# victorca25/traiNNer

Measured on AMD Instinct MI355X. Metric: HR images/sec (G+D step), ESRGAN x4 128->512, higher is better.
Workload: dtype f32 (bf16x3)

## Files before the change

### trainner_amd/csrc/wgrad_tile.hip

```cpp
#include <type_traits>
#include <utility>
#include "common.h"

namespace {

struct WgJob {
    const float *x; const float *g; float *ws; float *dbp;
    int x_ct, x_co, Cin, g_ct, g_co, Cout;
    int KoutP, KinVP;
    int cinp32;
    int ncib, job_begin;
};
struct WgK {
    int N, H, W, Ho, Wo;
    int tiles_x, tiles_y, tiles_total, tiles_per_split, nsplits, njobs;
    int bf;
    int reflect;
    WgJob job[TNR_WGRAD_GROUP_MAX];
};

template <int A_T, int B_T, int NTAPS_>
struct WgCfg {
    static constexpr int AB = A_T * B_T;
    static constexpr int KS = (NTAPS_ == 9 && (AB == 1 || AB == 2)) ? 4 / AB : 1;
// ... 102 lines not shown
        t_boff[j] = (ty * WT + tx) * CIB + bb * 32;
    }

    f32x16 acc[J];
#pragma unroll
    for (int j = 0; j < J; ++j)
#pragma unroll
        for (int r = 0; r < 16; ++r) acc[j][r] = 0.f;
    float bsum = 0.f;
    const bool want_bias = (a.dbp != nullptr) && (cib == 0);

    const int t_begin = split * a.tiles_per_split;
    int t_end = t_begin + a.tiles_per_split;
    if (t_end > a.tiles_total) t_end = a.tiles_total;

    constexpr int G_ITEMS = PX * (COB / 4), G_IT = (G_ITEMS + 255) / 256;
    constexpr int X_ITEMS = HT * WT * (CIB / 4), X_IT = (X_ITEMS + 255) / 256;
    constexpr int N_IT = G_IT + X_IT;
    constexpr int BATCH = (PIPE || N_IT <= 12) ? N_IT : 8;
    constexpr int NBATCH = (N_IT + BATCH - 1) / BATCH;
    f32x4 rr[BATCH];
    struct TileAt { int n, ty0, tx0; };
    auto tile_at = [&](int tile) __attribute__((always_inline)) {
        int q = tile;
        const int tx = q % a.tiles_x;
        q /= a.tiles_x;
        const int ty = q % a.tiles_y;
        return TileAt{q / a.tiles_y, ty * THG, tx * TWG};
    };
    auto load_item = [&](const TileAt &ta, int batch, auto kc) __attribute__((always_inline)) {
        constexpr int k = decltype(kc)::value;
        const int n = ta.n, ty0 = ta.ty0, tx0 = ta.tx0;
        {
            const int it = batch * BATCH + k;
            f32x4 v = {0.f, 0.f, 0.f, 0.f};
            if (it < G_IT) {
                const int i = tid + it * 256;
                const int p = i / (COB / 4), c4 = i - p * (COB / 4);
                const int r = p / TWG, c = p - r * TWG;
                const int oy = ty0 + r, ox = tx0 + c;
                const int co = cob * COB + c4 * 4;
                if (i < G_ITEMS && oy < a.Ho && ox < a.Wo && co < a.Cout) {
                    const int off = ((n * a.Ho + oy) * a.Wo + ox) * a.g_ct + a.g_co + co;
                    v = *reinterpret_cast<const f32x4 *>(a.g + off);
                }
            } else if (it < N_IT) {
                const int i = tid + (it - G_IT) * 256;
                const int pix = i / (CIB / 4), c4 = i - pix * (CIB / 4);
                const int hr = pix / WT, hc = pix - hr * WT;
                const int vb = cib * B_T + (c4 >> 3);
                int Y, X, c;
                bool ok;
                if (S2D) {
                    const int nb32 = a.cinp32 >> 5;
                    const int pp = vb / nb32;
                    c = (vb - pp * nb32) * 32 + (c4 & 7) * 4;
                    Y = 2 * (ty0 + hr) - 1 + (pp >> 1);
                    X = 2 * (tx0 + hc) - 1 + (pp & 1);
                    ok = (pp < 4) & (Y >= 0) & (Y < a.H) & (X >= 0) & (X < a.W);
                } else if (UP) {
                    c = vb * 32 + (c4 & 7) * 4;
                    Y = ty0 + hr - 1;
                    X = tx0 + hc - 1;
                    ok = (Y >= 0) & (Y < 2 * a.H) & (X >= 0) & (X < 2 * a.W);
                    Y >>= 1;
                    X >>= 1;
                } else {
                    c = vb * 32 + (c4 & 7) * 4;
                    Y = ty0 + hr - 1;
                    X = tx0 + hc - 1;
                    if (a.reflect) {
                        Y = Y < 0 ? -Y : (Y >= a.H ? 2 * a.H - 2 - Y : Y);
                        X = X < 0 ? -X : (X >= a.W ? 2 * a.W - 2 - X : X);
                    }
                    ok = (Y >= 0) & (Y < a.H) & (X >= 0) & (X < a.W);
                }
                if (i < X_ITEMS && ok && c < a.Cin) {
                    const int off = ((n * a.H + Y) * a.W + X) * a.x_ct + a.x_co + c;
                    v = *reinterpret_cast<const f32x4 *>(a.x + off);
                }
            }
            rr[k] = v;
        }
    };
    auto load_batch = [&](int tile, int batch) __attribute__((always_inline)) {
        const TileAt ta = tile_at(tile);
        wg_static_for<0, BATCH>([&](auto kc) __attribute__((always_inline)) { load_item(ta, batch, kc); });
    };
#if defined(TNR_WG_SPREAD_ALL) && !defined(TNR_NO_LOAD_SPREAD)
    constexpr bool SPREAD = PIPE;
#else
    constexpr bool SPREAD = false;
#endif
    constexpr int SPREAD_N = 3, IPG = (BATCH + SPREAD_N - 1) / SPREAD_N;
    auto load_group = [&](int tile, auto gc) __attribute__((always_inline)) {
        constexpr int g = decltype(gc)::value;
        constexpr int k0 = g * IPG < BATCH ? g * IPG : BATCH, k1 = (g + 1) * IPG < BATCH ? (g + 1) * IPG : BATCH;
        const TileAt ta = tile_at(tile);
        wg_static_for<k0, k1>([&](auto kc) __attribute__((always_inline)) { load_item(ta, 0, kc); });
    };
    auto split4 = [&](const f32x4 v, wg_f32x2 (&out)[3]) {
        wg_bf16x4 h, m, l;
#pragma unroll
        for (int i = 0; i < 4; ++i) {
            const __bf16 hh = (__bf16)v[i];
            const float r1 = v[i] - (float)hh;
            const __bf16 mm = (__bf16)r1;
            h[i] = hh;
            m[i] = mm;
            l[i] = (__bf16)(r1 - (float)mm);
        }
        out[0] = __builtin_bit_cast(wg_f32x2, h);
        out[1] = __builtin_bit_cast(wg_f32x2, m);
        out[2] = __builtin_bit_cast(wg_f32x2, l);
    };
    char *const s_gb = reinterpret_cast<char *>(smem);
    char *const s_xb = s_gb + (size_t)PX * COB * 6;
    auto store_batch = [&](int batch) {
#pragma unroll
        for (int k = 0; k < BATCH; ++k) {
            const int it = batch * BATCH + k;
            if constexpr (BF == 2) {
                wg_f32x2 pc[3];
                if (it < G_IT) {
                    const int i = tid + it * 256;
                    if (i < G_ITEMS) {
                        split4(rr[k], pc);
                        char *d = s_gb + wg_x3_off(i / (COB / 4), (i % (COB / 4)) * 4, COB);
#pragma unroll
                        for (int sp = 0; sp < 3; ++sp) *reinterpret_cast<wg_f32x2 *>(d + 256 * sp) = pc[sp];
                    }
                } else if (it < N_IT) {
                    const int i = tid + (it - G_IT) * 256;
                    if (i < X_ITEMS) {
                        split4(rr[k], pc);
                        char *d = s_xb + wg_x3_off(i / (CIB / 4), (i % (CIB / 4)) * 4, CIB);
#pragma unroll
                        for (int sp = 0; sp < 3; ++sp) *reinterpret_cast<wg_f32x2 *>(d + 256 * sp) = pc[sp];
                    }
                }
                continue;
            }
            if (it < G_IT) {
                const int i = tid + it * 256;
                if (i < G_ITEMS) *reinterpret_cast<f32x4 *>(s_g + i * 4) = rr[k];
            } else if (it < N_IT) {
                const int i = tid + (it - G_IT) * 256;
                if (i < X_ITEMS) *reinterpret_cast<f32x4 *>(s_x + i * 4) = rr[k];
            }
        }
    };

    if constexpr (DB) {
        static_assert(BF == 2 && MODE == TNR_CONV_3x3 && WPS == 1, "pipelined form: bf16x3, plain 3x3, one workgroup per CU");
        constexpr int WTP = 20;
        constexpr int G_BYTES = PX * COB * 6, X_BYTES = HT * WTP * CIB * 6, TILES_BYTES = G_BYTES + X_BYTES;
        constexpr int SET_BYTES = TILES_BYTES + 3072;
        constexpr int XBLK = (CIB / 32) * 768, GBLK = (COB / 32) * 768;
        constexpr int NP = (J + 1) / 2, MPR = 6 * J, NM = ROWS * MPR;
        constexpr int G0 = NM - 5 * N_IT - 6;
        static_assert(G0 >= 2 * N_IT, "the phase is too short for the staging plan");
        char *const lds = reinterpret_cast<char *>(smem);
        const __amdgpu_buffer_rsrc_t g_rs = __builtin_amdgcn_make_buffer_rsrc(const_cast<float *>(a.g), 0,
                                                                              (int)((unsigned)a.N * a.Ho * a.Wo * a.g_ct * 4u), 0x00020000);
        const __amdgpu_buffer_rsrc_t x_rs = __builtin_amdgcn_make_buffer_rsrc(const_cast<float *>(a.x), 0,
                                                                              (int)((unsigned)a.N * a.H * a.W * a.x_ct * 4u), 0x00020000);
        int it_src[N_IT], it_yx[N_IT], it_dst[N_IT];
#pragma unroll
        for (int k = 0; k < N_IT; ++k) {
            if (k < G_IT) {
                const int i = tid + k * 256;
                const int pp = i / (COB / 4), c4 = i - pp * (COB / 4);
                const int r = pp / TWG, cc = pp - r * TWG;
                const int co = cob * COB + c4 * 4;
                const bool v = i < G_ITEMS && co < a.Cout;
                it_src[k] = v ? (r * a.Wo + cc) * a.g_ct + a.g_co + co : -1;
                it_yx[k] = r | (cc << 8);
                it_dst[k] = i < G_ITEMS ? wg_x3_off(pp, c4 * 4, COB) : TILES_BYTES + tid * 8;
            } else {
                const int i = tid + (k - G_IT) * 256;
                const int pix = i / (CIB / 4), c4 = i - pix * (CIB / 4);
                const int hr = pix / WT, hc = pix - hr * WT;
                const int ch = (cib * B_T + (c4 >> 3)) * 32 + (c4 & 7) * 4;
                const bool v = i < X_ITEMS && ch < a.Cin;
                it_src[k] = v ? ((hr - 1) * a.W + (hc - 1)) * a.x_ct + a.x_co + ch : (1 << 30);
                it_yx[k] = hr | (hc << 8);
                it_dst[k] = i < X_ITEMS ? G_BYTES + wg_x3_off(hr * WTP + hc, c4 * 4, CIB) : TILES_BYTES + tid * 8;
            }
        }
        int ld_ty0 = 0, ld_tx0 = 0, ld_gbase = 0, ld_xbase = 0;
        bool ld_valid = true;
        int l_n = 0, l_ty = 0, l_tx = 0;
        auto load_setup_first = [&](int tile) __attribute__((always_inline)) {
            const TileAt ta = tile_at(tile);
            l_n = ta.n; l_ty = ta.ty0 / THG; l_tx = ta.tx0 / TWG;
        };
        auto load_setup_next = [&]() __attribute__((always_inline)) {
            if (++l_tx == a.tiles_x) {
                l_tx = 0;
                if (++l_ty == a.tiles_y) {
                    l_ty = 0;
                    ++l_n;
                }
            }
        };
        auto load_setup = [&]() __attribute__((always_inline)) {
            ld_ty0 = l_ty * THG; ld_tx0 = l_tx * TWG;
            ld_gbase = ((l_n * a.Ho + ld_ty0) * a.Wo + ld_tx0) * a.g_ct;
            ld_xbase = ((l_n * a.H + ld_ty0) * a.W + ld_tx0) * a.x_ct;
        };
        auto item_load = [&](auto kc) __attribute__((always_inline)) {
            constexpr int k = decltype(kc)::value;
            const int y = it_yx[k] & 255, xx = it_yx[k] >> 8;
            if constexpr (k < G_IT) {
                const bool ok = ld_valid & (it_src[k] >= 0) & (ld_ty0 + y < a.Ho) & (ld_tx0 + xx < a.Wo);
                const unsigned bo = ok ? (unsigned)(ld_gbase + it_src[k]) * 4u : 0xfffffff0u;
                rr[k] = __builtin_bit_cast(f32x4, __builtin_amdgcn_raw_buffer_load_b128(g_rs, (int)bo, 0, 0));
            } else {
                const int Y = ld_ty0 + y - 1, X = ld_tx0 + xx - 1;
                const bool ok = ld_valid & (it_src[k] != (1 << 30)) & ((unsigned)Y < (unsigned)a.H) & ((unsigned)X < (unsigned)a.W);
                const unsigned bo = ok ? (unsigned)(ld_xbase + it_src[k]) * 4u : 0xfffffff0u;
                rr[k] = __builtin_bit_cast(f32x4, __builtin_amdgcn_raw_buffer_load_b128(x_rs, (int)bo, 0, 0));
            }
        };
        wg_bf16x4 ih, im, il;
        f32x4 ir;
        auto item_step = [&](auto kc, auto sc, char *set) __attribute__((always_inline)) {
            constexpr int k = decltype(kc)::value, st = decltype(sc)::value;
            if constexpr (st == 0) {
#if WG_PK_SPLIT
                wg_pk_level(rr[k], ih, ir);
#else
                ih = __builtin_convertvector(rr[k], wg_bf16x4);
                ir = rr[k] - __builtin_convertvector(ih, f32x4);
#endif
            } else if constexpr (st == 1) {
#if WG_PK_SPLIT
                const f32x4 r1 = ir;
                wg_pk_level(r1, im, ir);
#else
                im = __builtin_convertvector(ir, wg_bf16x4);
                ir = ir - __builtin_convertvector(im, f32x4);
#endif
            } else {
#if WG_PK_SPLIT
                if constexpr (st == 2) {
                    const wg_f32x2 a = {ir[0], ir[1]}, b = {ir[2], ir[3]};
                    il = __builtin_bit_cast(wg_bf16x4, wg_f32x2{__builtin_bit_cast(float, __builtin_convertvector(a, wg_bf16x2)),
                                                                __builtin_bit_cast(float, __builtin_convertvector(b, wg_bf16x2))});
                }
#else
                if constexpr (st == 2) il = __builtin_convertvector(ir, wg_bf16x4);
#endif
                *reinterpret_cast<wg_f32x2 *>(set + it_dst[k] + 256 * (st - 2)) = __builtin_bit_cast(wg_f32x2, st == 2 ? ih : (st == 3 ? im : il));
            }
        };
        const int cg = (lane >> 4) & 1, m4 = (lane >> 2) & 3, q4 = lane & 3;
        const int lch = 16 * cg + 4 * q4;
        const int ga_off = ((pg * ROWS * 4 + 2 * half) * (COB / 32) + aa_w) * 768 + m4 * 64 + lch * 2;
        int xb_off[J];
#pragma unroll
        for (int j = 0; j < J; ++j) {
            const int tap = t_tap[j] >> 10, bb = t_tap[j] & 31;
            const int ty = tap / KH, tx = tap - ty * KH;
            const int q0 = tx + 8 * half + m4;
            xb_off[j] = G_BYTES + ((pg * ROWS + ty) * (WTP / 4) + (q0 >> 2)) * XBLK + (q0 & 3) * 64 + bb * 768 + lch * 2;
        }
        constexpr int TA[6] = {0, 2, 1, 0, 1, 0}, TB[6] = {2, 0, 1, 1, 0, 0};
        auto rd = [&](const char *base, int imm) __attribute__((always_inline)) {
            return __builtin_amdgcn_ds_read_tr16_b64_v4i16((wg_lds_s16x4 *)(base + imm));
        };
        typedef short s16x8 __attribute__((ext_vector_type(8)));
        static_assert(J == 9 && WPG == AB, "every wave owns the 9 taps of one (cout half, cin block) pair: tile j = tap j");
        wg_s16x4 ra[2][3][2], rbx[3][3][3][2];
        auto pack = [&](const wg_s16x4 lo4, const wg_s16x4 hi4) __attribute__((always_inline)) {
            const s16x8 v = {lo4[0], lo4[1], lo4[2], lo4[3], hi4[0], hi4[1], hi4[2], hi4[3]};
            return __builtin_bit_cast(wg_bf16x8, v);
        };

        if (t_begin < t_end) {
            load_setup_first(t_begin);
            load_setup();
            wg_static_for<0, N_IT>([&](auto kc) __attribute__((always_inline)) { item_load(kc); });
            wg_static_for<0, N_IT>([&](auto kc) __attribute__((always_inline)) {
                wg_static_for<0, 5>([&](auto sc) __attribute__((always_inline)) { item_step(kc, sc, lds); });
            });
            __syncthreads();
        }
        for (int tile = t_begin; tile < t_end; ++tile) {
            const int cur = (tile - t_begin) & 1;
            const char *set = lds + cur * SET_BYTES;
            char *oset = lds + (cur ^ 1) * SET_BYTES;
            ld_valid = tile + 1 < t_end;
            if (ld_valid) load_setup_next();
            load_setup();
            const char *gab = set + ga_off;
            const char *xbb[3];
#pragma unroll
            for (int j = 0; j < 3; ++j) xbb[j] = set + xb_off[j];
            auto read_a = [&](auto rc, auto idc) __attribute__((always_inline)) {
                constexpr int r = decltype(rc)::value, id = decltype(idc)::value, sp = id >> 1, hh = id & 1;
                ra[r & 1][sp][hh] = rd(gab, r * 4 * GBLK + 256 * sp + hh * GBLK);
            };
            auto read_x = [&](auto xrc, auto txc, auto idc) __attribute__((always_inline)) {
                constexpr int xr = decltype(xrc)::value, tx = decltype(txc)::value, id = decltype(idc)::value, sp = id >> 1, hh = id & 1;
                rbx[xr % 3][tx][sp][hh] = rd(xbb[tx], xr * 5 * XBLK + 256 * sp + hh * XBLK);
            };
            if (tile == t_begin) {
                wg_static_for<0, 6>([&](auto idc) __attribute__((always_inline)) { read_a(std::integral_constant<int, 0>{}, idc); });
                wg_static_for<0, 6>([&](auto idc) __attribute__((always_inline)) { read_x(std::integral_constant<int, 0>{}, std::integral_constant<int, 0>{}, idc); });
                wg_static_for<0, 6>([&](auto idc) __attribute__((always_inline)) { read_x(std::integral_constant<int, 0>{}, std::integral_constant<int, 1>{}, idc); });
            }
            const char *gab_n = oset + ga_off;
            const char *xbb_n[2] = {oset + xb_off[0], oset + xb_off[1]};
            auto read_next = [&](auto idc) __attribute__((always_inline)) {
                constexpr int id = decltype(idc)::value;
                if constexpr (id < 6) {
                    constexpr int sp = id >> 1, hh = id & 1;
                    ra[0][sp][hh] = rd(gab_n, 256 * sp + hh * GBLK);
                } else {
                    constexpr int tx = (id - 6) / 6, k = (id - 6) % 6, sp = k >> 1, hh = k & 1;
                    rbx[0][tx][sp][hh] = rd(xbb_n[tx], 256 * sp + hh * XBLK);
                }
            };
            __builtin_amdgcn_sched_barrier(0);
            wg_static_for<0, ROWS>([&](auto rc) __attribute__((always_inline)) {
                constexpr int r = decltype(rc)::value;
                wg_static_for<0, NP>([&](auto jpc) __attribute__((always_inline)) {
                    constexpr int jp = decltype(jpc)::value;
                    constexpr int j0 = 2 * jp, nt = (j0 + 1 < J) ? 2 : 1, nm = 6 * nt;
                    constexpr int gbase = r * MPR + jp * 12;
                    constexpr int nj0 = 2 * (jp + 1), nnt = (nj0 + 1 < J) ? 2 : 1;
                    constexpr int NRD = (r == 0 && jp + 1 < NP) ? (6 * nnt + ((jp + 2 == NP && ROWS > 1) ? 6 : 0)) : 0;
                    constexpr int RDEN = nm > 5 ? nm - 4 : 2, RPH = (NRD + RDEN - 1) / RDEN;
                    wg_bf16x8 fa[3], fbv[2][3];
#pragma unroll
                    for (int sp = 0; sp < 3; ++sp) {
                        fa[sp] = pack(ra[r & 1][sp][0], ra[r & 1][sp][1]);
#pragma unroll
                        for (int q = 0; q < nt; ++q) fbv[q][sp] = pack(rbx[(r + (j0 + q) / 3) % 3][(j0 + q) % 3][sp][0], rbx[(r + (j0 + q) / 3) % 3][(j0 + q) % 3][sp][1]);
                    }
                    static_assert(((ROWS - 1) & 1) == 1, "the next tile's gradient fragment goes into register set 0");
                    if constexpr (r + 1 == ROWS && jp + 1 == NP) __syncthreads();
                    if constexpr (jp == 0) {
                        if (want_bias) {
#pragma unroll
                            for (int kk = 0; kk < 8; ++kk) bsum += ((float)fa[0][kk] + (float)fa[1][kk]) + (float)fa[2][kk];
                        }
                    }
                    __builtin_amdgcn_sched_barrier(0);
                    wg_static_for<0, nm>([&](auto ic) __attribute__((always_inline)) {
                        constexpr int i = decltype(ic)::value, pq = nt == 2 ? i / 2 : i, q = nt == 2 ? i % 2 : 0;
                        constexpr int g = gbase + i;
                        acc[j0 + q] = __builtin_amdgcn_mfma_f32_32x32x16_bf16(fa[TA[pq]], fbv[q][TB[pq]], acc[j0 + q], 0, 0, 0);
                        if constexpr (r + 1 == ROWS && jp + 1 == NP) {
                            wg_static_for<0, 3>([&](auto kc) __attribute__((always_inline)) { read_next(std::integral_constant<int, 3 * i + decltype(kc)::value>{}); });
                        }
                        if constexpr (r == 0) {
                            wg_static_for<0, RPH>([&](auto kc) __attribute__((always_inline)) {
                                constexpr int id = i * RPH + decltype(kc)::value;
                                if constexpr (id < NRD) {
                                    if constexpr (id < 6 * nnt) {
                                        constexpr int jn = nj0 + id / 6;
                                        read_x(std::integral_constant<int, jn / 3>{}, std::integral_constant<int, jn % 3>{}, std::integral_constant<int, id % 6>{});
                                    } else {
                                        read_a(std::integral_constant<int, 1>{}, std::integral_constant<int, id - 6 * nnt>{});
                                    }
                                }
                            });
                        } else {
                            constexpr int m = jp * 12 + i;
                            if constexpr (m < 18) read_x(std::integral_constant<int, r + 2>{}, std::integral_constant<int, (m < 18 ? m / 6 : 0)>{}, std::integral_constant<int, m % 6>{});
                            else if constexpr (m < 24 && r + 1 < ROWS) read_a(std::integral_constant<int, (r + 1 < ROWS ? r + 1 : r)>{}, std::integral_constant<int, (m >= 18 && m < 24 ? m - 18 : 0)>{});
                        }
#ifndef WG_ABL_NOITEMS
                        if constexpr ((g & 1) == 0 && g / 2 < N_IT) {
                            item_load(std::integral_constant<int, (g / 2 < N_IT ? g / 2 : 0)>{});
                        }
                        if constexpr (g >= G0 && g < G0 + 5 * N_IT) {
                            item_step(std::integral_constant<int, (g >= G0 && g < G0 + 5 * N_IT ? (g - G0) / 5 : 0)>{},
                                      std::integral_constant<int, (g >= G0 ? (g - G0) % 5 : 0)>{}, oset);
                        }
#endif
                        __builtin_amdgcn_sched_barrier(0);
                    });
                });
            });
        }
        __syncthreads();
    } else {
    if (PIPE && t_begin < t_end) load_batch(t_begin, 0);
        for (int tile = t_begin; tile < t_end; ++tile) {
            if (PIPE) {
                __syncthreads();
                store_batch(0);
                __syncthreads();
                if (!SPREAD && tile + 1 < t_end) load_batch(tile + 1, 0);
            } else {
                load_batch(tile, 0);
                __syncthreads();
                store_batch(0);
    #pragma unroll
                for (int bt = 1; bt < NBATCH; ++bt) {
                    load_batch(tile, bt);
                    store_batch(bt);
                }
                __syncthreads();
            }
            {
                int go = half * COB + li + aa_w * 32 + pg * ROWS * TWG * COB;
                int xo[J];
    #pragma unroll
                for (int j = 0; j < J; ++j) xo[j] = PX * COB + half * CIB + li + t_boff[j] + pg * ROWS * WT * CIB;
                if constexpr (BF == 2) {
                    constexpr int NP = (J + 1) / 2;
                    constexpr int TA[6] = {0, 2, 1, 0, 1, 0}, TB[6] = {2, 0, 1, 1, 0, 0};
                    const int cg = (lane >> 4) & 1, m4 = (lane >> 2) & 3, q4 = lane & 3;
                    const int lch = 16 * cg + 4 * q4;
                    auto frag = [&](const char *base, wg_bf16x8 (&out)[3], int rd_stride) {
    #pragma unroll
                        for (int sp = 0; sp < 3; ++sp) {
                            const wg_s16x4 lo4 = __builtin_amdgcn_ds_read_tr16_b64_v4i16((wg_lds_s16x4 *)(base + 256 * sp));
                            const wg_s16x4 hi4 = __builtin_amdgcn_ds_read_tr16_b64_v4i16((wg_lds_s16x4 *)(base + 256 * sp + rd_stride));
                            typedef short s16x8 __attribute__((ext_vector_type(8)));
                            const s16x8 v = {lo4[0], lo4[1], lo4[2], lo4[3], hi4[0], hi4[1], hi4[2], hi4[3]};
                            out[sp] = __builtin_bit_cast(wg_bf16x8, v);
                        }
                    };
                    const char *ga_ptr = s_gb + ((pg * ROWS * 4 + 2 * half) * (COB / 32) + aa_w) * 768 + m4 * 64 + lch * 2;
                    constexpr int GA_ROW = 4 * (COB / 32) * 768, GA_RD = (COB / 32) * 768, XB_RD = (CIB / 32) * 768;
                    int xpix[J], xblk[J];
                    const int lpix = 8 * half + m4, lblk = lch * 2;
    #pragma unroll
                    for (int j = 0; j < J; ++j) {
                        const int tap = t_tap[j] >> 10, bb = t_tap[j] & 31;
                        const int ty = tap / KH, tx = tap - ty * KH;
                        xpix[j] = __builtin_amdgcn_readfirstlane((pg * ROWS + ty) * WT + tx);
                        xblk[j] = __builtin_amdgcn_readfirstlane(bb * 768);
                    }
                    auto xaddr = [&](int j) {
                        const int P = xpix[j] + lpix;
                        return s_xb + (P >> 2) * ((CIB / 32) * 768) + (P & 3) * 64 + xblk[j] + lblk;
                    };
                    constexpr int NSET = WPS == 1 ? 2 : 1;
                    wg_bf16x8 ca[3], cb[NSET][2][3];
                    auto read_pair = [&](int jp, int set) {
    #pragma unroll
                        for (int q = 0; q < 2; ++q) {
                            const int j = 2 * jp + q < J ? 2 * jp + q : J - 1;
                            frag(xaddr(j), cb[set][q], XB_RD);
                        }
                    };
    #pragma unroll 1
                    for (int r = 0; r < ROWS; ++r) {
                        frag(ga_ptr, ca, GA_RD);
                        if (NSET == 2) read_pair(0, 0);
                        if (want_bias) {
    #pragma unroll
                            for (int kk = 0; kk < 8; ++kk) bsum += ((float)ca[0][kk] + (float)ca[1][kk]) + (float)ca[2][kk];
                        }
    #pragma unroll
                        for (int jp = 0; jp < NP; ++jp) {
                            if (NSET == 1) read_pair(jp, 0);
                            else if (jp + 1 < NP) read_pair(jp + 1, (jp + 1) & 1);
                            __builtin_amdgcn_sched_barrier(0);
                            const int cs = NSET == 1 ? 0 : (jp & 1);
    #pragma unroll
                            for (int p = 0; p < 6; ++p) {
                                acc[2 * jp] = __builtin_amdgcn_mfma_f32_32x32x16_bf16(ca[TA[p]], cb[cs][0][TB[p]], acc[2 * jp], 0, 0, 0);
                                if (2 * jp + 1 < J)
                                    acc[2 * jp + 1] = __builtin_amdgcn_mfma_f32_32x32x16_bf16(ca[TA[p]], cb[cs][1][TB[p]], acc[2 * jp + 1], 0, 0, 0);
                            }
                            __builtin_amdgcn_sched_barrier(0);
                        }
                        ga_ptr += GA_ROW;
    #pragma unroll
                        for (int j = 0; j < J; ++j) xpix[j] += WT;
                    }
                } else if constexpr (BF) {
                    float ra[8], rb[8][J];
                    wg_bf16x8 ca, cb[J];
                    auto read_row = [&]() {
    #pragma unroll
                        for (int kk = 0; kk < 8; ++kk) {
                            ra[kk] = smem[go + 2 * kk * COB];
    #pragma unroll
                            for (int j = 0; j < J; ++j) rb[kk][j] = smem[xo[j] + 2 * kk * CIB];
                        }
                    };
                    auto pack_row = [&]() {
    #pragma unroll
                        for (int kk = 0; kk < 8; ++kk) {
                            bsum += ra[kk];
                            ca[kk] = (__bf16)ra[kk];
    #pragma unroll
                            for (int j = 0; j < J; ++j) cb[j][kk] = (__bf16)rb[kk][j];
                        }
                    };
                    read_row();
                    pack_row();
    #pragma unroll 1
                    for (int r = 0; r < ROWS; ++r) {
                        go += TWG * COB;
    #pragma unroll
                        for (int j = 0; j < J; ++j) xo[j] += WT * CIB;
                        if (r + 1 < ROWS) read_row();
                        if constexpr (SPREAD) {
                            if (tile + 1 < t_end) {
                                if constexpr (ROWS >= SPREAD_N) {
                                    if (r == 0) load_group(tile + 1, std::integral_constant<int, 0>{});
                                    if (r == 1) load_group(tile + 1, std::integral_constant<int, 1>{});
// ... 57 lines not shown
            if (pg == p) {
#pragma unroll
                for (int j = 0; j < J; ++j)
#pragma unroll
                    for (int r = 0; r < 16; ++r) smem[((wq * J + j) * 16 + r) * 64 + lane] = acc[j][r];
                smem[ACC_FLOATS + wq * 64 + lane] = btot;
            }
            __syncthreads();
            if (pg == 0) {
#pragma unroll
                for (int j = 0; j < J; ++j)
#pragma unroll
                    for (int r = 0; r < 16; ++r) acc[j][r] += smem[((wq * J + j) * 16 + r) * 64 + lane];
                btot += smem[ACC_FLOATS + wq * 64 + lane];
            }
        }
        if (pg != 0) return;
    }

    {
        const int nblk = a.KinVP >> 5;
        const int nsl = a.nsplits, sl = split;
        const size_t row_stride = (size_t)nblk * nsl * 32;
#pragma unroll
        for (int j = 0; j < J; ++j) {
            const int tap = t_tap[j] >> 10, aa = (t_tap[j] >> 5) & 31, bb = t_tap[j] & 31;
            const int blk = cib * B_T + bb;
            const int co0 = cob * COB + aa * 32;
            if (!t_ok[j] || blk >= nblk || co0 >= a.KoutP) continue;
            float *p = a.ws + (((size_t)tap * a.KoutP + co0 + 4 * half) * nblk + blk) * nsl * 32 + (size_t)sl * 32 + li;
#pragma unroll
            for (int r = 0; r < 16; ++r) p[(size_t)((r & 3) + 8 * (r >> 2)) * row_stride] = acc[j][r];
        }
    }
    if (want_bias && wq < AB && (wq % B_T) == 0) {
        const int co = cob * COB + aa_w * 32 + li;
        if (half == 0 && co < a.KoutP) a.dbp[(size_t)co * a.nsplits + split] = btot;
    }
}

struct RedJob {
    const float *ws; const float *dbp; float *dw; float *db;
    float *dw2; float *db2;
    int split, cin_total2;
    int KoutP, KinVP, cinp32, Cout, Cin, cin_total, cin_begin;
    int blk_begin, nrows;
    float alpha, beta;
};
struct RedK {
    int splits, ntaps, kh, kw, s2d, njobs;
    int rpb;
    RedJob job[TNR_WGRAD_GROUP_MAX];
};

__global__ void __launch_bounds__(256) wgrad_reduce_kernel(const RedK ga) {
    __shared__ float sh[8][33];
    int ji = 0;
#pragma unroll
    for (int q = 1; q < TNR_WGRAD_GROUP_MAX; ++q)
        if (q < ga.njobs && (int)blockIdx.x >= ga.job[q].blk_begin) ji = q;
    const RedJob &a = ga.job[ji];
    const int bx = (int)blockIdx.x - a.blk_begin;
    const int splits = ga.splits;
    const int nblk = a.KinVP >> 5;
    const int el = threadIdx.x & 31, sl = threadIdx.x >> 5;
    const int nrows = a.nrows;
    const int nrowblk = (nrows + ga.rpb - 1) / ga.rpb;
    if (bx >= nrowblk) {
        const int c = (bx - nrowblk) * 32 + el;
        float part = 0.f;
        if (c < a.Cout)
            for (int q = sl; q < splits; q += 8) part += a.dbp[(size_t)c * splits + q];
        sh[sl][el] = part;
        __syncthreads();
        if (sl == 0 && c < a.Cout) {
            float sum = 0.f;
#pragma unroll
            for (int l = 0; l < 8; ++l) sum += sh[l][el];
            float *dbc = c < a.split ? a.db + c : a.db2 + (c - a.split);
            const float prev = (a.beta != 0.f) ? a.beta * *dbc : 0.f;
            *dbc = prev + a.alpha * sum;
        }
        return;
    }
    const int row = ga.rpb == 8 ? bx * 8 + sl : bx;
    if (row >= nrows) return;
    const int blk = row % nblk;
    const int co = (row / nblk) % a.KoutP;
    const int tap = row / (nblk * a.KoutP);
    const float *src = a.ws + (size_t)row * splits * 32 + el;
    float p0 = 0.f, p1 = 0.f, p2 = 0.f, p3 = 0.f;
    float sum_all = 0.f;
    if (ga.rpb == 8) {
        float q[8] = {0.f, 0.f, 0.f, 0.f, 0.f, 0.f, 0.f, 0.f};
        int s8 = 0;
        for (; s8 + 8 <= splits; s8 += 8) {
#pragma unroll
            for (int k = 0; k < 8; ++k) q[k] += src[(size_t)(s8 + k) * 32];
        }
#pragma unroll
        for (int k = 0; k < 8; ++k)
            if (s8 + k < splits) q[k] += src[(size_t)(s8 + k) * 32];
        sum_all = ((q[0] + q[1]) + (q[2] + q[3])) + ((q[4] + q[5]) + (q[6] + q[7]));
    }
    int s = ga.rpb == 8 ? splits : sl;
    for (; s + 24 < splits; s += 32) {
        p0 += src[(size_t)s * 32];
        p1 += src[(size_t)(s + 8) * 32];
        p2 += src[(size_t)(s + 16) * 32];
        p3 += src[(size_t)(s + 24) * 32];
    }
    for (; s < splits; s += 8) p0 += src[(size_t)s * 32];
    if (ga.rpb != 8) {
        sh[sl][el] = (p0 + p1) + (p2 + p3);
        __syncthreads();
    }
    if (sl == 0 || ga.rpb == 8) {
        float sum = sum_all;
        if (ga.rpb != 8) {
#pragma unroll
            for (int l = 0; l < 8; ++l) sum += sh[l][el];
        }
        const int civ = blk * 32 + el;
        int ci, ky, kx;
        if (ga.s2d) {
            const int pp = civ / a.cinp32;
            ci = civ - pp * a.cinp32;
            ky = 2 * (tap >> 1) + (pp >> 1);
            kx = 2 * (tap & 1) + (pp & 1);
        } else {
            ci = civ;
            ky = tap / ga.kw;
            kx = tap - ky * ga.kw;
        }
        if (co < a.Cout && ci < a.Cin) {
            const bool second = co >= a.split;
            const size_t o = (((size_t)(second ? co - a.split : co) * (second ? a.cin_total2 : a.cin_total) + a.cin_begin + ci) * ga.kh + ky) * ga.kw + kx;
            float *dst = (second ? a.dw2 : a.dw) + o;
            const float prev = (a.beta != 0.f) ? a.beta * *dst : 0.f;
            *dst = prev + a.alpha * sum;
        }
    }
}

struct WgPlan {
    int a_t, b_t, thg, ks, wps, db;
    int ncib, ncob;
    int KoutP, KinVP, cinp32;
    int tiles_x, tiles_y, tiles_total, splits, tiles_per_split;
    int ntaps, resident;
    int64_t ws_floats, db_floats;
};

int plan_wgrad(const tnr_wgrad_desc *d, WgPlan &p, int group_jobs) {
    const bool s2d = d->mode == TNR_CONV_4x4_S2;
    p.a_t = d->Cout > 32 ? 2 : 1;
    const int vch = s2d ? 4 * tnr_round_up(d->Cin, 32) : tnr_round_up(d->Cin, 32);
    const int vblocks = vch / 32;
    if (p.a_t == 2) {
        p.b_t = vblocks >= 2 ? 2 : 1;
    } else {
        p.b_t = vblocks >= 4 ? 4 : vblocks;
        if (vblocks == 5) p.b_t = 3;
    }
    p.thg = (p.a_t == 2 || p.b_t <= 2 || (p.b_t == 4 && d->mode != TNR_CONV_4x4_S2)) ? 8 : 4;
    const int ab = p.a_t * p.b_t;
    p.ks = (!s2d && (ab == 1 || ab == 2)) ? 4 / ab : 1;
    if (p.ks > 1) p.thg = 16;
    if (p.ks > 1 && d->mma == TNR_MMA_BF16X3 && p.a_t == 1 && p.b_t == 2) p.thg = 8;
    const int wpg0 = 4 / p.ks;
    p.wps = ((p.a_t * p.b_t * (s2d ? 4 : 9) + wpg0 - 1) / wpg0 >= 9) ? 1 : 2;
    static const int x3_occ = [] { const char *e = getenv("TNR_WG_X3_OCC"); return e ? atoi(e) : 3; }();
    p.db = 0;
    if (d->mma == TNR_MMA_BF16X3 && s2d && x3_occ >= 2 && p.a_t == 2 && p.b_t == 2) p.thg = 4;
    if (d->mma == TNR_MMA_BF16X3 && !s2d && x3_occ >= 2 && p.wps == 1) {
        if (p.b_t == 4) p.b_t = 2;
        const int ab2 = p.a_t * p.b_t;
        p.ks = (ab2 == 1 || ab2 == 2) ? 4 / ab2 : 1;
        p.thg = ab2 == 1 ? 8 : 4;
        p.wps = 2;
        if (x3_occ == 3 && d->mode == TNR_CONV_3x3 && d->pad_mode == 0 && p.b_t <= 2 &&
            (int64_t)d->N * d->H * d->W * d->x.ctot < (1LL << 30) && (int64_t)d->N * d->Ho * d->Wo * d->g.ctot < (1LL << 30)) {
            p.wps = 1;
            p.db = 1;
        }
    }
    p.cinp32 = tnr_round_up(d->Cin, 32);
    p.KinVP = vch;
    p.KoutP = tnr_round_up(d->Cout, 32);
    p.ncib = tnr_cdiv(vblocks, p.b_t);
    p.ncob = tnr_cdiv(p.KoutP, 32 * p.a_t);
    p.ntaps = s2d ? 4 : 9;
    p.tiles_x = tnr_cdiv(d->Wo, 16);
    p.tiles_y = tnr_cdiv(d->Ho, p.thg);
    p.tiles_total = p.tiles_x * p.tiles_y * d->N;
    p.resident = 256 * p.wps;
    const int jobs = group_jobs > 0 ? group_jobs : p.ncib * p.ncob;
    int want = p.resident / jobs;
    if (want < 1) want = 1;
    int max_splits = tnr_cdiv(p.tiles_total, 4);
    if (max_splits < 1) max_splits = 1;
    p.splits = want < max_splits ? want : max_splits;
    if (p.splits < 1) p.splits = 1;
    p.tiles_per_split = tnr_cdiv(p.tiles_total, p.splits);
    p.splits = tnr_cdiv(p.tiles_total, p.tiles_per_split);
    p.ws_floats = (int64_t)p.splits * p.ntaps * p.KoutP * p.KinVP;
    p.db_floats = (int64_t)p.splits * p.KoutP;
    return 0;
}

template <int MODE, int A_T, int B_T, int THG, int BF, int WPS = WgCfg<A_T, B_T, (MODE == TNR_CONV_4x4_S2 ? 4 : 9)>::WAVES_PER_SIMD, bool DB = false>
int launch_wgrad_t(const WgK &k, int jobs, hipStream_t s) {
    constexpr int KH = (MODE == TNR_CONV_4x4_S2) ? 2 : 3;
    constexpr size_t lds_f32 = (size_t)(THG * 16 * 32 * A_T + (THG + KH) * (16 + KH - 1) * 32 * B_T) * sizeof(float);
    constexpr size_t lds_x3 = (size_t)(THG * 16 * 32 * A_T + (((THG + KH - 1) * (16 + KH - 1) + 3) / 4) * 4 * 32 * B_T) * 6;
    using Cfg = WgCfg<A_T, B_T, (MODE == TNR_CONV_4x4_S2 ? 4 : 9)>;
    constexpr size_t lds_red = Cfg::KS > 1 ? (size_t)(Cfg::WPG * Cfg::J * 16 * 64 + Cfg::WPG * 64) * sizeof(float) : 0;
    constexpr size_t lds_db = 2 * ((size_t)(THG * 16 * 32 * A_T + (THG + KH - 1) * 20 * 32 * B_T) * 6 + 3072);
    constexpr size_t lds_tile = DB ? lds_db : (BF == 2 ? lds_x3 : lds_f32);
    constexpr size_t lds = lds_tile > lds_red ? lds_tile : lds_red;
    constexpr bool one_wg = WPS == 1;
    if constexpr (BF == 2 && lds > 160 * 1024) {
        tnr_set_error("wgrad_tile: tile class %d x %d x %d rows does not fit the LDS in TNR_MMA_BF16X3", A_T, B_T, THG);
        return TNR_EINVAL;
    } else {
    static_assert(lds <= ((one_wg || BF == 2) ? 160 : 80) * 1024, "wgrad tile exceeds the LDS budget of its occupancy regime");
    static bool attr_done = false;
    auto fn = wgrad_tile_kernel<MODE, A_T, B_T, THG, BF, WPS, DB>;
    if (!attr_done) {
        if (hipFuncSetAttribute(reinterpret_cast<const void *>(fn), hipFuncAttributeMaxDynamicSharedMemorySize, (int)lds) !=
            hipSuccess) {
            tnr_set_error("wgrad_tile: cannot raise dynamic LDS to %zu bytes", lds);
            return TNR_ELAUNCH;
        }
        attr_done = true;
    }
    hipLaunchKernelGGL(fn, dim3(k.nsplits, jobs, 1), dim3(256), lds, s, k);
    return tnr_check_launch("wgrad_tile");
    }
}

template <int MODE, int A_T, int B_T, int THG>
int launch_wgrad(const WgK &k, int jobs, hipStream_t s) {
    if (k.bf == 2) return launch_wgrad_t<MODE, A_T, B_T, THG, 2>(k, jobs, s);
    return k.bf ? launch_wgrad_t<MODE, A_T, B_T, THG, 1>(k, jobs, s) : launch_wgrad_t<MODE, A_T, B_T, THG, 0>(k, jobs, s);
}

template <int MODE>
int dispatch_wgrad(const WgK &k, const WgPlan &p, int jobs, hipStream_t s) {
    constexpr int THS = (MODE == TNR_CONV_4x4_S2) ? 8 : 16;
    if constexpr (MODE == TNR_CONV_3x3) {
        if (k.bf == 2 && p.db) {
            if (p.a_t == 2) return p.b_t == 2 ? launch_wgrad_t<MODE, 2, 2, 4, 2, 1, true>(k, jobs, s) : launch_wgrad_t<MODE, 2, 1, 4, 2, 1, true>(k, jobs, s);
            return p.b_t == 2 ? launch_wgrad_t<MODE, 1, 2, 4, 2, 1, true>(k, jobs, s) : launch_wgrad_t<MODE, 1, 1, 8, 2, 1, true>(k, jobs, s);
        }
    }
    if constexpr (MODE != TNR_CONV_4x4_S2) {
        if (k.bf == 2 && p.wps == 2 && p.b_t <= 2) {
            if (p.a_t == 2) return p.b_t == 2 ? launch_wgrad_t<MODE, 2, 2, 4, 2, 2>(k, jobs, s) : launch_wgrad_t<MODE, 2, 1, 4, 2, 2>(k, jobs, s);
            return p.b_t == 2 ? launch_wgrad_t<MODE, 1, 2, 4, 2, 2>(k, jobs, s) : launch_wgrad_t<MODE, 1, 1, 8, 2, 2>(k, jobs, s);
        }
    }
    if (p.a_t == 2) {
        if constexpr (MODE == TNR_CONV_4x4_S2) {
            if (p.b_t == 2 && k.bf == 2 && p.thg == 4) return launch_wgrad_t<MODE, 2, 2, 4, 2, 2>(k, jobs, s);
        }
        if (p.b_t == 2) return launch_wgrad<MODE, 2, 2, 8>(k, jobs, s);
        return launch_wgrad<MODE, 2, 1, THS>(k, jobs, s);
    }
    switch (p.b_t) {
        case 1: return launch_wgrad<MODE, 1, 1, THS>(k, jobs, s);
        case 2:
            if constexpr (MODE != TNR_CONV_4x4_S2) {
                if (p.thg == 8) return launch_wgrad_t<MODE, 1, 2, 8, 2>(k, jobs, s);
            }
            return launch_wgrad<MODE, 1, 2, THS>(k, jobs, s);
        case 3: return launch_wgrad<MODE, 1, 3, 4>(k, jobs, s);
        default:
            if constexpr (MODE != TNR_CONV_4x4_S2) {
                if (p.thg == 8) return launch_wgrad<MODE, 1, 4, 8>(k, jobs, s);
            }
            return launch_wgrad<MODE, 1, 4, 4>(k, jobs, s);
    }
}

int check_wgrad_desc(const tnr_wgrad_desc *d) {
    TNR_REQUIRE(d->x.ptr && d->g.ptr && d->dw && d->ws, "wgrad: null pointer");
    TNR_REQUIRE(d->mode == TNR_CONV_3x3 || d->mode == TNR_CONV_3x3_UP2 || d->mode == TNR_CONV_4x4_S2,
                "wgrad: bad mode %d", d->mode);
    TNR_REQUIRE((d->x.ctot % 4) == 0 && (d->x.coff % 4) == 0 && (d->g.ctot % 4) == 0 && (d->g.coff % 4) == 0,
                "wgrad: views must be 4-channel aligned");
    TNR_REQUIRE(d->db == nullptr || d->cin_begin == 0, "wgrad: bias gradient only with cin_begin == 0");
    if (d->cout_split != 0) {
        TNR_REQUIRE(d->cout_split > 0 && d->cout_split < d->Cout && d->cout_split % 32 == 0 && d->dw2 != nullptr && d->cin_total2 >= d->cin_begin + d->Cin,
                    "wgrad: bad cout pair (split %d of %d output channels)", d->cout_split, d->Cout);
        TNR_REQUIRE((d->db == nullptr) == (d->db2 == nullptr), "wgrad: a cout pair takes both bias gradients or none");
    }
    if (d->mode == TNR_CONV_3x3) TNR_REQUIRE(d->Ho == d->H && d->Wo == d->W, "wgrad3x3: size mismatch");
    if (d->mode == TNR_CONV_3x3_UP2) TNR_REQUIRE(d->Ho == 2 * d->H && d->Wo == 2 * d->W, "wgrad3x3_up2: size mismatch");
    if (d->mode == TNR_CONV_4x4_S2) TNR_REQUIRE(2 * d->Ho == d->H && 2 * d->Wo == d->W, "wgrad4x4s2: size mismatch");
    TNR_REQUIRE((int64_t)d->N * d->H * d->W * d->x.ctot < (1LL << 31) && (int64_t)d->N * d->Ho * d->Wo * d->g.ctot < (1LL << 31),
                "wgrad: buffers above 2^31 elements need 64-bit offsets");
    return TNR_OK;
}

}

extern "C" int64_t tnr_wgrad_workspace_bytes(const tnr_wgrad_desc *d) {
    if (d == nullptr) return 0;
    WgPlan p;
    plan_wgrad(d, p, 0);
    return (p.ws_floats + p.db_floats) * (int64_t)sizeof(float);
}

extern "C" int tnr_conv_wgrad_group(const tnr_wgrad_desc *descs, int32_t n, void *stream) {
    TNR_REQUIRE(descs != nullptr && n >= 1 && n <= TNR_WGRAD_GROUP_MAX, "wgrad_group: 1..%d layers per group", TNR_WGRAD_GROUP_MAX);
    WgPlan plans[TNR_WGRAD_GROUP_MAX];
    int jobs = 0;
    for (int i = 0; i < n; ++i) {
        const int rc = check_wgrad_desc(&descs[i]);
        if (rc != TNR_OK) return rc;
        plan_wgrad(&descs[i], plans[i], 0);
        jobs += plans[i].ncib * plans[i].ncob;
        const tnr_wgrad_desc &d0 = descs[0], &di = descs[i];
        TNR_REQUIRE(di.mode == d0.mode && di.N == d0.N && di.H == d0.H && di.W == d0.W && di.Ho == d0.Ho && di.Wo == d0.Wo,
                    "wgrad_group: layer %d does not share the pixel geometry of layer 0", i);
        TNR_REQUIRE(plans[i].a_t == plans[0].a_t && plans[i].b_t == plans[0].b_t && plans[i].thg == plans[0].thg && plans[i].ks == plans[0].ks && plans[i].db == plans[0].db,
                    "wgrad_group: layer %d (%d->%d channels) is not in the tile class of layer 0 (%d->%d)", i, di.Cin,
                    di.Cout, d0.Cin, d0.Cout);
    }
    TNR_REQUIRE(jobs <= 65535, "wgrad_group: too many channel blocks");
    WgK k;
    RedK r;
    static const int red_rpb = [] { const char *e = getenv("TNR_WGRAD_REDUCE_RPB"); return e ? atoi(e) : 8; }();
    WgPlan pg = plans[0];
    if (n > 1) plan_wgrad(&descs[0], pg, jobs);
    const int rpb = (red_rpb == 8 && pg.splits <= 32) ? 8 : 1;
    int job_begin = 0, blk_begin = 0;
    for (int i = 0; i < n; ++i) {
        const tnr_wgrad_desc *d = &descs[i];
        WgPlan &p = plans[i];
        if (n > 1) plan_wgrad(d, p, jobs);
        TNR_REQUIRE(p.splits == plans[0].splits && p.tiles_per_split == plans[0].tiles_per_split, "wgrad_group: split mismatch");
        TNR_REQUIRE((p.ws_floats + p.db_floats) * (int64_t)sizeof(float) <= d->ws_bytes,
                    "wgrad: workspace too small (%lld < %lld)", (long long)d->ws_bytes,
                    (long long)((p.ws_floats + p.db_floats) * sizeof(float)));
        for (int q = 0; q < i; ++q) TNR_REQUIRE(descs[q].ws != d->ws, "wgrad_group: layers %d and %d share a workspace", q, i);
        WgJob &j = k.job[i];
        j.x = d->x.ptr; j.x_ct = d->x.ctot; j.x_co = d->x.coff; j.Cin = d->Cin;
        j.g = d->g.ptr; j.g_ct = d->g.ctot; j.g_co = d->g.coff; j.Cout = d->Cout;
        j.ws = d->ws; j.dbp = d->db ? d->ws + p.ws_floats : nullptr;
        j.KoutP = p.KoutP; j.KinVP = p.KinVP; j.cinp32 = p.cinp32;
        j.ncib = p.ncib; j.job_begin = job_begin;
        job_begin += p.ncib * p.ncob;
        RedJob &q = r.job[i];
        q.ws = d->ws; q.dbp = j.dbp; q.dw = d->dw; q.db = d->db;
        q.dw2 = d->dw2; q.db2 = d->db2; q.split = d->cout_split > 0 ? d->cout_split : d->Cout; q.cin_total2 = d->cin_total2;
        q.KoutP = p.KoutP; q.KinVP = p.KinVP; q.cinp32 = p.cinp32; q.Cout = d->Cout; q.Cin = d->Cin;
        q.cin_total = d->cin_total; q.cin_begin = d->cin_begin; q.alpha = d->alpha; q.beta = d->beta;
        q.blk_begin = blk_begin;
        q.nrows = p.ntaps * p.KoutP * (p.KinVP / 32);
        blk_begin += tnr_cdiv(q.nrows, rpb) + (d->db ? tnr_cdiv(d->Cout, 32) : 0);
    }
    for (int i = n; i < TNR_WGRAD_GROUP_MAX; ++i) { k.job[i] = k.job[0]; r.job[i] = r.job[0]; }
    const tnr_wgrad_desc &d0 = descs[0];
    const WgPlan &p0 = plans[0];
    k.N = d0.N; k.H = d0.H; k.W = d0.W; k.Ho = d0.Ho; k.Wo = d0.Wo;
    k.tiles_x = p0.tiles_x; k.tiles_y = p0.tiles_y; k.tiles_total = p0.tiles_total;
    k.tiles_per_split = p0.tiles_per_split; k.nsplits = p0.splits; k.njobs = n;
    TNR_REQUIRE(d0.mma >= TNR_MMA_F32 && d0.mma <= TNR_MMA_BF16X3, "wgrad: bad mma %d", d0.mma);
    k.bf = d0.mma;
    k.reflect = d0.pad_mode == 1;
    TNR_REQUIRE(d0.pad_mode == 0 || (d0.pad_mode == 1 && d0.mode == TNR_CONV_3x3 && d0.H >= 2 && d0.W >= 2), "wgrad: pad_mode 1 (reflection) is for TNR_CONV_3x3");
    for (int i = 1; i < n; ++i) TNR_REQUIRE(descs[i].pad_mode == d0.pad_mode, "wgrad_group: layer %d: one border mode per launch", i);
    for (int i = 1; i < n; ++i) TNR_REQUIRE(descs[i].mma == d0.mma, "wgrad_group: layer %d: one matrix-core precision per launch", i);
    hipStream_t s = (hipStream_t)stream;
    int rc;
    switch (d0.mode) {
        case TNR_CONV_3x3: rc = dispatch_wgrad<TNR_CONV_3x3>(k, p0, jobs, s); break;
        case TNR_CONV_3x3_UP2: rc = dispatch_wgrad<TNR_CONV_3x3_UP2>(k, p0, jobs, s); break;
        default: rc = dispatch_wgrad<TNR_CONV_4x4_S2>(k, p0, jobs, s); break;
    }
    if (rc != TNR_OK) return rc;
    r.splits = p0.splits; r.ntaps = p0.ntaps; r.s2d = d0.mode == TNR_CONV_4x4_S2;
    r.kh = r.s2d ? 4 : 3; r.kw = r.kh; r.njobs = n; r.rpb = rpb;
    hipLaunchKernelGGL(wgrad_reduce_kernel, dim3((unsigned)blk_begin), dim3(256), 0, s, r);
    return tnr_check_launch("wgrad_reduce");
}

extern "C" int tnr_conv_wgrad(const tnr_wgrad_desc *d, void *stream) {
    TNR_REQUIRE(d != nullptr, "wgrad: null descriptor");
    return tnr_conv_wgrad_group(d, 1, stream);
}
```

Baseline: 73.63.

## Extend pipelined bf16x3 wgrad kernel to stride-2 4x4 and upsample-3x3 convs

Generalizes the double-buffered, one-workgroup-per-CU weight-gradient kernel beyond plain 3x3 so it also serves 4x4 stride-2 (space-to-depth) and 2x-upsample 3x3 convolutions. The halo addressing, bounds checks, register arrays and LDS read schedule are adapted for KH=2 tap layouts and the upsampled/strided source coordinates. The planner enables this path by default for a_t=b_t=2 when offsets fit in 32 bits, with an env switch to disable it. The aim is to overlap global loads with MFMA work for these layers, at the cost of lower occupancy and more complex indexing that could be wrong for edge shapes.

```diff
diff --git a/trainner_amd/csrc/wgrad_tile.hip b/trainner_amd/csrc/wgrad_tile.hip
--- a/trainner_amd/csrc/wgrad_tile.hip
+++ b/trainner_amd/csrc/wgrad_tile.hip
@@ -278,13 +278,15 @@
     };
 
     if constexpr (DB) {
-        static_assert(BF == 2 && MODE == TNR_CONV_3x3 && WPS == 1, "pipelined form: bf16x3, plain 3x3, one workgroup per CU");
+        static_assert(BF == 2 && WPS == 1, "pipelined form: bf16x3, one workgroup per CU");
+        static_assert(MODE != TNR_CONV_3x3_UP2 || THG % 2 == 0, "UP: even tile origins (a halo item is base + a constant offset)");
         constexpr int WTP = 20;
         constexpr int G_BYTES = PX * COB * 6, X_BYTES = HT * WTP * CIB * 6, TILES_BYTES = G_BYTES + X_BYTES;
         constexpr int SET_BYTES = TILES_BYTES + 3072;
         constexpr int XBLK = (CIB / 32) * 768, GBLK = (COB / 32) * 768;
         constexpr int NP = (J + 1) / 2, MPR = 6 * J, NM = ROWS * MPR;
-        constexpr int G0 = NM - 5 * N_IT - 6;
+        constexpr int NM_LAST = 6 * (J - 2 * (NP - 1));
+        constexpr int G0 = NM - 5 * N_IT - NM_LAST;
         static_assert(G0 >= 2 * N_IT, "the phase is too short for the staging plan");
         char *const lds = reinterpret_cast<char *>(smem);
         const __amdgpu_buffer_rsrc_t g_rs = __builtin_amdgcn_make_buffer_rsrc(const_cast<float *>(a.g), 0,
@@ -307,10 +309,24 @@
                 const int i = tid + (k - G_IT) * 256;
                 const int pix = i / (CIB / 4), c4 = i - pix * (CIB / 4);
                 const int hr = pix / WT, hc = pix - hr * WT;
-                const int ch = (cib * B_T + (c4 >> 3)) * 32 + (c4 & 7) * 4;
+                const int vb = cib * B_T + (c4 >> 3);
+                int ch, dy = hr, dx = hc, src;
+                if constexpr (S2D) {
+                    const int nb32 = a.cinp32 >> 5, pp = vb / nb32;
+                    ch = pp < 4 ? (vb - pp * nb32) * 32 + (c4 & 7) * 4 : a.Cin;
+                    dy = 2 * hr + (pp >> 1);
+                    dx = 2 * hc + (pp & 1);
+                    src = (dy - 1) * a.W + (dx - 1);
+                } else if constexpr (UP) {
+                    ch = vb * 32 + (c4 & 7) * 4;
+                    src = ((hr - 1) >> 1) * a.W + ((hc - 1) >> 1);
+                } else {
+                    ch = vb * 32 + (c4 & 7) * 4;
+                    src = (hr - 1) * a.W + (hc - 1);
+                }
                 const bool v = i < X_ITEMS && ch < a.Cin;
-                it_src[k] = v ? ((hr - 1) * a.W + (hc - 1)) * a.x_ct + a.x_co + ch : (1 << 30);
-                it_yx[k] = hr | (hc << 8);
+                it_src[k] = v ? src * a.x_ct + a.x_co + ch : (1 << 30);
+                it_yx[k] = dy | (dx << 8);
                 it_dst[k] = i < X_ITEMS ? G_BYTES + wg_x3_off(hr * WTP + hc, c4 * 4, CIB) : TILES_BYTES + tid * 8;
             }
         }
@@ -333,7 +349,8 @@
         auto load_setup = [&]() __attribute__((always_inline)) {
             ld_ty0 = l_ty * THG; ld_tx0 = l_tx * TWG;
             ld_gbase = ((l_n * a.Ho + ld_ty0) * a.Wo + ld_tx0) * a.g_ct;
-            ld_xbase = ((l_n * a.H + ld_ty0) * a.W + ld_tx0) * a.x_ct;
+            const int sy = S2D ? 2 * ld_ty0 : (UP ? ld_ty0 >> 1 : ld_ty0), sx = S2D ? 2 * ld_tx0 : (UP ? ld_tx0 >> 1 : ld_tx0);
+            ld_xbase = ((l_n * a.H + sy) * a.W + sx) * a.x_ct;
         };
         auto item_load = [&](auto kc) __attribute__((always_inline)) {
             constexpr int k = decltype(kc)::value;
@@ -343,8 +360,9 @@
                 const unsigned bo = ok ? (unsigned)(ld_gbase + it_src[k]) * 4u : 0xfffffff0u;
                 rr[k] = __builtin_bit_cast(f32x4, __builtin_amdgcn_raw_buffer_load_b128(g_rs, (int)bo, 0, 0));
             } else {
-                const int Y = ld_ty0 + y - 1, X = ld_tx0 + xx - 1;
-                const bool ok = ld_valid & (it_src[k] != (1 << 30)) & ((unsigned)Y < (unsigned)a.H) & ((unsigned)X < (unsigned)a.W);
+                const int Y = (S2D ? 2 * ld_ty0 : ld_ty0) + y - 1, X = (S2D ? 2 * ld_tx0 : ld_tx0) + xx - 1;
+                const int BH = UP ? 2 * a.H : a.H, BW = UP ? 2 * a.W : a.W;
+                const bool ok = ld_valid & (it_src[k] != (1 << 30)) & ((unsigned)Y < (unsigned)BH) & ((unsigned)X < (unsigned)BW);
                 const unsigned bo = ok ? (unsigned)(ld_xbase + it_src[k]) * 4u : 0xfffffff0u;
                 rr[k] = __builtin_bit_cast(f32x4, __builtin_amdgcn_raw_buffer_load_b128(x_rs, (int)bo, 0, 0));
             }
@@ -397,8 +415,8 @@
             return __builtin_amdgcn_ds_read_tr16_b64_v4i16((wg_lds_s16x4 *)(base + imm));
         };
         typedef short s16x8 __attribute__((ext_vector_type(8)));
-        static_assert(J == 9 && WPG == AB, "every wave owns the 9 taps of one (cout half, cin block) pair: tile j = tap j");
-        wg_s16x4 ra[2][3][2], rbx[3][3][3][2];
+        static_assert(J == NTAPS && WPG == AB, "every wave owns the taps of one (cout half, cin block) pair: tile j = tap j");
+        wg_s16x4 ra[2][3][2], rbx[3][KH][3][2];
         auto pack = [&](const wg_s16x4 lo4, const wg_s16x4 hi4) __attribute__((always_inline)) {
             const s16x8 v = {lo4[0], lo4[1], lo4[2], lo4[3], hi4[0], hi4[1], hi4[2], hi4[3]};
             return __builtin_bit_cast(wg_bf16x8, v);
@@ -421,9 +439,9 @@
             if (ld_valid) load_setup_next();
             load_setup();
             const char *gab = set + ga_off;
-            const char *xbb[3];
-#pragma unroll
-            for (int j = 0; j < 3; ++j) xbb[j] = set + xb_off[j];
+            const char *xbb[KH];
+#pragma unroll
+            for (int j = 0; j < KH; ++j) xbb[j] = set + xb_off[j];
             auto read_a = [&](auto rc, auto idc) __attribute__((always_inline)) {
                 constexpr int r = decltype(rc)::value, id = decltype(idc)::value, sp = id >> 1, hh = id & 1;
                 ra[r & 1][sp][hh] = rd(gab, r * 4 * GBLK + 256 * sp + hh * GBLK);
@@ -464,7 +482,7 @@
                     for (int sp = 0; sp < 3; ++sp) {
                         fa[sp] = pack(ra[r & 1][sp][0], ra[r & 1][sp][1]);
 #pragma unroll
-                        for (int q = 0; q < nt; ++q) fbv[q][sp] = pack(rbx[(r + (j0 + q) / 3) % 3][(j0 + q) % 3][sp][0], rbx[(r + (j0 + q) / 3) % 3][(j0 + q) % 3][sp][1]);
+                        for (int q = 0; q < nt; ++q) fbv[q][sp] = pack(rbx[(r + (j0 + q) / KH) % 3][(j0 + q) % KH][sp][0], rbx[(r + (j0 + q) / KH) % 3][(j0 + q) % KH][sp][1]);
                     }
                     static_assert(((ROWS - 1) & 1) == 1, "the next tile's gradient fragment goes into register set 0");
                     if constexpr (r + 1 == ROWS && jp + 1 == NP) __syncthreads();
@@ -480,9 +498,32 @@
                         constexpr int g = gbase + i;
                         acc[j0 + q] = __builtin_amdgcn_mfma_f32_32x32x16_bf16(fa[TA[pq]], fbv[q][TB[pq]], acc[j0 + q], 0, 0, 0);
                         if constexpr (r + 1 == ROWS && jp + 1 == NP) {
-                            wg_static_for<0, 3>([&](auto kc) __attribute__((always_inline)) { read_next(std::integral_constant<int, 3 * i + decltype(kc)::value>{}); });
-                        }
-                        if constexpr (r == 0) {
+                            constexpr int RN = (18 + nm - 1) / nm;
+                            wg_static_for<0, RN>([&](auto kc) __attribute__((always_inline)) {
+                                constexpr int id = RN * i + decltype(kc)::value;
+                                if constexpr (id < 18) read_next(std::integral_constant<int, id>{});
+                            });
+                        }
+                        if constexpr (KH == 2) {
+                            if constexpr (r == 0 && jp == 0) {
+                                wg_static_for<0, RPH>([&](auto kc) __attribute__((always_inline)) {
+                                    constexpr int id = i * RPH + decltype(kc)::value;
+                                    if constexpr (id < NRD) {
+                                        if constexpr (id < 6 * nnt) {
+                                            constexpr int jn = nj0 + id / 6;
+                                            read_x(std::integral_constant<int, jn / KH>{}, std::integral_constant<int, jn % KH>{}, std::integral_constant<int, id % 6>{});
+                                        } else {
+                                            read_a(std::integral_constant<int, 1>{}, std::integral_constant<int, id - 6 * nnt>{});
+                                        }
+                                    }
+                                });
+                            } else if constexpr (jp == 0) {
+                                if constexpr (i < 6 && r + 1 < ROWS) read_a(std::integral_constant<int, (r + 1 < ROWS ? r + 1 : r)>{}, std::integral_constant<int, (i < 6 ? i : 0)>{});
+                            }
+                            if constexpr (jp == 1 && r + 1 < ROWS) {
+                                read_x(std::integral_constant<int, r + 2>{}, std::integral_constant<int, i / 6>{}, std::integral_constant<int, i % 6>{});
+                            }
+                        } else if constexpr (r == 0) {
                             wg_static_for<0, RPH>([&](auto kc) __attribute__((always_inline)) {
                                 constexpr int id = i * RPH + decltype(kc)::value;
                                 if constexpr (id < NRD) {
@@ -846,6 +887,11 @@
     int64_t ws_floats, db_floats;
 };
 
+bool wg_s2_db() {
+    const char *e = getenv("TNR_WG_S2_DB");
+    return !(e && atoi(e) == 0);
+}
+
 int plan_wgrad(const tnr_wgrad_desc *d, WgPlan &p, int group_jobs) {
     const bool s2d = d->mode == TNR_CONV_4x4_S2;
     p.a_t = d->Cout > 32 ? 2 : 1;
@@ -867,6 +913,8 @@
     static const int x3_occ = [] { const char *e = getenv("TNR_WG_X3_OCC"); return e ? atoi(e) : 3; }();
     p.db = 0;
     if (d->mma == TNR_MMA_BF16X3 && s2d && x3_occ >= 2 && p.a_t == 2 && p.b_t == 2) p.thg = 4;
+    const bool fits32 = (int64_t)d->N * d->H * d->W * d->x.ctot < (1LL << 30) && (int64_t)d->N * d->Ho * d->Wo * d->g.ctot < (1LL << 30);
+    if (d->mma == TNR_MMA_BF16X3 && s2d && x3_occ == 3 && p.a_t == 2 && p.b_t == 2 && fits32 && wg_s2_db()) p.db = 1;
     if (d->mma == TNR_MMA_BF16X3 && !s2d && x3_occ >= 2 && p.wps == 1) {
         if (p.b_t == 4) p.b_t = 2;
         const int ab2 = p.a_t * p.b_t;
@@ -878,6 +926,7 @@
             p.wps = 1;
             p.db = 1;
         }
+        if (x3_occ == 3 && d->mode == TNR_CONV_3x3_UP2 && p.a_t == 2 && p.b_t == 2 && fits32 && wg_s2_db()) p.db = 1;
     }
     p.cinp32 = tnr_round_up(d->Cin, 32);
     p.KinVP = vch;
@@ -948,6 +997,8 @@
             if (p.a_t == 2) return p.b_t == 2 ? launch_wgrad_t<MODE, 2, 2, 4, 2, 1, true>(k, jobs, s) : launch_wgrad_t<MODE, 2, 1, 4, 2, 1, true>(k, jobs, s);
             return p.b_t == 2 ? launch_wgrad_t<MODE, 1, 2, 4, 2, 1, true>(k, jobs, s) : launch_wgrad_t<MODE, 1, 1, 8, 2, 1, true>(k, jobs, s);
         }
+    } else {
+        if (k.bf == 2 && p.db) return launch_wgrad_t<MODE, 2, 2, 4, 2, 1, true>(k, jobs, s);
     }
     if constexpr (MODE != TNR_CONV_4x4_S2) {
         if (k.bf == 2 && p.wps == 2 && p.b_t <= 2) {
```

Result: no change. 74.03, median of 6 (+0.5%).
